# abowman6/CBET_RayTracing_3D

Hardware: AMD Instinct MI355X
Metric: ray-steps/sec, OMEGA 60-beam 256^3 sweep (higher is better)
Workload: dtype f64

## Files before the change

### cbet_raytracing_3d_amd/csrc/cbet_relocate.h

```cpp
#ifndef CBET_RELOCATE_H_
#define CBET_RELOCATE_H_

#include <math.h>

#include "cbet_hd.h"

namespace cbet {

CBET_HD int relocate_loop(int c, double f, int n)
{
    const double half = 0.5001;
    int q = (n - 1 < c + 1) ? n - 1 : c + 1;
    while (q >= ((0 > c - 1) ? 0 : c - 1)) {
        c = (fabs(q - f) < half) ? q : c;
        --q;
    }
    return c;
}

CBET_HD int relocate_closed(int c, double f, int n)
{
    const double half = 0.5001;
    const double fc = (double)c;
    const bool up = (c + 1 <= n - 1) && (fabs((fc + 1.0) - f) < half);
    const bool mid = fabs(fc - f) < half;
    const bool dn1 = (c - 1 >= 0) && (fabs((fc - 1.0) - f) < half);
    const bool dn2 = (c - 2 >= 0) && (fabs((fc - 2.0) - f) < half);
    const int lower = dn1 ? (dn2 ? c - 2 : c - 1) : c;
    const int upper = mid ? c : c + 1;
    return up ? upper : lower;
}

constexpr int kRelocateDeep = 6;
CBET_HD int relocate_deep_interior(int c, double fc, double f, bool &far)
{
    const double half = 0.5001;
    const double g = f - fc;
    far = far || !(fabs(g) < 1.4998);
    return c + ((g >= half) ? 1 : 0) - ((g < (half - 1.0)) ? 1 : 0);
}

}
#endif
```

### cbet_raytracing_3d_amd/csrc/cbet_trace_diag.h

```cpp
#ifndef CBET_TRACE_DIAG_H_
#define CBET_TRACE_DIAG_H_

#include "cbet_trace_common.h"

namespace cbet {

#ifdef CBET_DIAG_CLOCKS
#define CBET_IF_CLOCKS(...) __VA_ARGS__
#else
#define CBET_IF_CLOCKS(...)
#endif
#ifdef CBET_DIAG_FACES
#define CBET_IF_FACES(...) __VA_ARGS__
#else
#define CBET_IF_FACES(...)
#endif
#ifdef CBET_DIAG_CHAIN
#define CBET_IF_CHAIN(...) __VA_ARGS__
#else
#define CBET_IF_CHAIN(...)
#endif

struct WaveDiag {
    typedef unsigned long long u64;
    static constexpr bool kCountsWaveSteps = (0 CBET_IF_CLOCKS(+1) CBET_IF_FACES(+1) CBET_IF_CHAIN(+1)) != 0;
    CBET_IF_CLOCKS(u64 wait = 0, arm = 0, n_arm = 0, ret = 0, n_ret = 0, t_start, t_wait, t_arm, t_ret;)
    CBET_IF_FACES(unsigned near_steps = 0, near_axes = 0, arm_steps = 0;)
    CBET_IF_CHAIN(u64 chain = 0, t_chain = 0;)

    static __device__ __forceinline__ void stamp(u64 &t) { asm volatile("s_memtime %0" : "=&s"(t) : : "memory"); }
    static __device__ __forceinline__ void stamp_wait(u64 &t) { asm volatile("s_memtime %0\n\ts_waitcnt lgkmcnt(0)" : "=&s"(t) : : "memory"); }
    static __device__ __forceinline__ u64 since(u64 t0)
    {
        u64 t1;
        asm volatile("s_memtime %0\n\ts_waitcnt lgkmcnt(0)" : "=&s"(t1) : "s"(t0) : "memory");
        return t1 - t0;
    }

    __device__ __forceinline__ void begin() { CBET_IF_CLOCKS(stamp_wait(t_start);) }
    __device__ __forceinline__ void step_begin(int near)
    {
        (void)near;
        CBET_IF_FACES(near_steps += near != 0 ? 1 : 0; near_axes += __builtin_popcount((unsigned)near);)
    }
    __device__ __forceinline__ void wait_begin() { CBET_IF_CLOCKS(stamp(t_wait);) }
    __device__ __forceinline__ void wait_end()
    {
        CBET_IF_CLOCKS(wait += since(t_wait);)
        CBET_IF_CHAIN(stamp_wait(t_chain);)
    }
    __device__ __forceinline__ void chain_end() { CBET_IF_CHAIN(chain += since(t_chain);) }
    __device__ __forceinline__ void arm_begin()
    {
        CBET_IF_FACES(arm_steps += 1;)
        CBET_IF_CLOCKS(stamp(t_arm);)
    }
    __device__ __forceinline__ void arm_end() { CBET_IF_CLOCKS(arm += since(t_arm); n_arm += 1;) }
    __device__ __forceinline__ void retire_begin() { CBET_IF_CLOCKS(stamp(t_ret);) }
    __device__ __forceinline__ void retire_end() { CBET_IF_CLOCKS(ret += since(t_ret); n_ret += 1;) }
    __device__ __forceinline__ bool report(const TraceArgs &a, int lane, int tot_steps, int tot_rays, unsigned wave_steps)
    {
        auto put = [&](int slot, u64 v) { atomicAdd(&a.counters[slot], v); };
        if (kCountsWaveSteps && lane == 0) {
            CBET_IF_CLOCKS(u64 t_end; stamp_wait(t_end);)
            put(kCntSteps, (u64)tot_steps);
            put(kCntWaveSteps, (u64)wave_steps);
#if defined(CBET_DIAG_CLOCKS)
            put(kCntGlobalAtomics, wait);
            put(kCntEvictions, arm);
            put(kCntWaveStepsWide, n_arm);
            put(kCntSlabsRetired, t_end - t_start);
            put(kCntRays, ret);
            put(kCntWaveStepsMiss, n_ret);
#elif defined(CBET_DIAG_CHAIN)
            put(kCntRays, (u64)tot_rays);
            put(kCntGlobalAtomics, chain);
#elif defined(CBET_DIAG_FACES)
            put(kCntRays, (u64)tot_rays);
            put(kCntWaveStepsWide, (u64)near_steps);
            put(kCntWaveStepsMiss, (u64)near_axes);
            put(kCntSlabsRetired, (u64)arm_steps);
#endif
        }
        (void)tot_rays;
        return kCountsWaveSteps;
    }
};
#undef CBET_IF_CLOCKS
#undef CBET_IF_FACES
#undef CBET_IF_CHAIN

}

#endif
```

### cbet_raytracing_3d_amd/csrc/cbet_trace_window.hip

```cpp
#include <hip/hip_runtime.h>

#include <cstddef>
#include <type_traits>

#if defined(__HIP_DEVICE_COMPILE__) && !defined(__gfx950__)
#error "cbet_trace_window.hip is written for gfx950 (CDNA4) only"
#endif

#include "cbet_trace_common.h"
#include "cbet_trace_diag.h"

namespace cbet {
namespace {

#define CBET_BALLOT(cond) __builtin_amdgcn_ballot_w64(cond)
#define CBET_LANES(mask) __builtin_amdgcn_inverse_ballot_w64(mask)
#define CBET_USUAL(cond) __builtin_expect(!!(cond), 1)
#define CBET_RARE(cond) __builtin_expect(!!(cond), 0)
#define CBET_SELDOM(cond) __builtin_expect_with_probability(!!(cond), 0, 0.9)

template <int WX_, int WY_, int WZ_, bool PAD, bool XORSW = false>
struct Tile {
    static constexpr int WX = WX_, WY = WY_, WZ = WZ_;
    static constexpr int XM = WX - 1, YM = WY - 1, ZM = WZ - 1;
    static constexpr bool ROT = PAD && WZ == 16;
    static constexpr int YS = (PAD && !ROT) ? WZ + 1 : WZ;
    static constexpr int XS = (PAD && !ROT) ? WY * YS + 4 : WY * WZ;
    static constexpr bool XOR = ROT && XORSW;
    static __device__ __forceinline__ int zr(int tx, int ty, int tz)
    {
        return XOR ? (tz ^ ((tx & 3) << 2) ^ (ty << 1)) : (ROT ? ((tz + 7 * tx + 3 * ty) & ZM) : tz);
    }
    static_assert(!XOR || (WX == 8 && WY == 8 && WZ == 16), "the swizzle terms are written for the 8 x 8 x 16 box");
    static __device__ __forceinline__ int xterm(int tx) { return __mul24(tx, XS * 8 + 32) & ~0x80; }
    static __device__ __forceinline__ int yterm(int ty) { return __mul24(ty, YS * 8 + 16); }
    static constexpr int N = WX * XS;
    static constexpr int SX = WX - 2, SY = WY - 2, SZ = WZ - 2;
    static constexpr bool BRICK = WZ == 16 && WY == 8;
    static constexpr int DT = WX * WY * WZ;
    static __device__ __forceinline__ int slot_d(int tx, int ty, int tz) { return (tx * WY + ty) * WZ + tz; }
};

struct Origin {
    int x, y, z;
};

template <int M>
__device__ __forceinline__ int abs_in(int o, int r) { return o + ((r - o) & M); }

template <int C>
struct Corner {
    static constexpr int index = C;
    template <class V> static __device__ __forceinline__ V x(V v0, V v1) { return (C & 1) ? v1 : v0; }
    template <class V> static __device__ __forceinline__ V z(V v0, V v1) { return (C & 2) ? v1 : v0; }
    template <class V> static __device__ __forceinline__ V y(V v0, V v1) { return (C & 4) ? v1 : v0; }
};
template <class F>
__device__ __forceinline__ void each_corner(F f)
{
    f(Corner<0>{}); f(Corner<1>{}); f(Corner<2>{}); f(Corner<3>{}); f(Corner<4>{}); f(Corner<5>{}); f(Corner<6>{}); f(Corner<7>{});
}

struct WaveCounters {
    int n_atomics = 0;
    int n_miss = 0;
    unsigned steps_miss = 0;
    unsigned slabs_bsteps = 0;
    int pend = 0;
    [[no_unique_address]] WaveDiag dg;
};
struct PairedMissCounters : WaveCounters {};

constexpr unsigned long long kEvenLanes = 0x5555555555555555ull;
__device__ __forceinline__ unsigned long long pair_owners(unsigned long long hbm_m, int round)
{
    return hbm_m & (round == 0 ? kEvenLanes : ~kEvenLanes);
}
__device__ __forceinline__ unsigned long long pair_lanes(unsigned long long owners, int round)
{
    return owners | (round == 0 ? owners << 1 : owners >> 1);
}
__device__ __forceinline__ int pair_issued(unsigned long long hbm_m)
{
    return (pair_owners(hbm_m, 0) != 0ull ? 4 : 0) + (pair_owners(hbm_m, 1) != 0ull ? 4 : 0);
}
#define CBET_PAIR_DPP " quad_perm:[1,0,3,2] row_mask:0xf bank_mask:0xf bound_ctrl:1"
__device__ __forceinline__ int pair_pick(unsigned long long owners, int mine, int lent)
{
    int r;
    asm volatile("s_nop 1\n\ts_mov_b64 vcc, %1\n\tv_cndmask_b32_dpp %0, %2, %3, vcc" CBET_PAIR_DPP
                 : "=&v"(r) : "s"(owners), "v"(lent), "v"(mine) : "vcc");
    return r;
}
__device__ __forceinline__ void pair_pick(unsigned long long owners, int mine_n, int lent_n, double mine_v, double lent_v, int &n, double &v)
{
    int lo, hi;
    asm volatile("s_nop 1\n\ts_mov_b64 vcc, %3\n\t"
                 "v_cndmask_b32_dpp %0, %4, %5, vcc" CBET_PAIR_DPP "\n\t"
                 "v_cndmask_b32_dpp %1, %6, %7, vcc" CBET_PAIR_DPP "\n\t"
                 "v_cndmask_b32_dpp %2, %8, %9, vcc" CBET_PAIR_DPP
                 : "=&v"(n), "=&v"(lo), "=&v"(hi)
                 : "s"(owners), "v"(lent_n), "v"(mine_n), "v"(__double2loint(lent_v)), "v"(__double2loint(mine_v)),
                   "v"(__double2hiint(lent_v)), "v"(__double2hiint(mine_v))
                 : "vcc");
    v = __hiloint2double(hi, lo);
}

template <bool W32>
struct Grid {
    double *p;
};
template <bool W32>
__device__ __forceinline__ void grid_add(const TraceArgs &a, Grid<W32> g, int node, double v)
{
    if constexpr (W32) global_add(a, reinterpret_cast<double *>(reinterpret_cast<char *>(g.p) + ((unsigned)node * 8u)), v);
    else global_add(a, &g.p[node], v);
}
template <bool W32>
__device__ __forceinline__ void grid_add_far(const TraceArgs &a, Grid<W32> g, long index, double v) { global_add(a, &g.p[index], v); }

template <class G>
__device__ __forceinline__ void write_back(const TraceArgs &a, double *tile, int slot, G edep, int node, double v, WaveCounters &wc)
{
    wc.pend += (CBET_BALLOT(v != 0.0) != 0ull) ? 1 : 0;
    if (v != 0.0) {
        tile[slot] = 0.0;
        ++wc.n_atomics;
        grid_add(a, edep, node, v);
    }
}
template <class G>
__device__ __forceinline__ void write_back_far(const TraceArgs &a, double *tile, int slot, G edep, long index, double v, WaveCounters &wc)
{
    wc.pend += (CBET_BALLOT(v != 0.0) != 0ull) ? 1 : 0;
    if (v != 0.0) {
        grid_add_far(a, edep, index, v);
        tile[slot] = 0.0;
        ++wc.n_atomics;
    }
}

template <class WC, class F>
__device__ __forceinline__ void miss_add8(unsigned long long hbm_m, WC &wc, F add8)
{
    constexpr bool PAIRED = std::is_same<WC, PairedMissCounters>::value;
    if (CBET_RARE(hbm_m != 0ull)) {
        wc.pend += PAIRED ? pair_issued(hbm_m) : 8;
        if (PAIRED || CBET_LANES(hbm_m)) add8();
    }
}

template <class T, int AX, int COUNT, class G>
__device__ __forceinline__ void retire_planes(const TraceArgs &a, double *tile, const Origin &o, int coord, int step,
                                              int lane, G edep, int sXh, int sYh, WaveCounters &wc)
{
    constexpr int WO = AX == 0 ? T::WY : T::WX, OM = WO - 1;
    constexpr int IT = (WO * T::WZ + kWave - 1) / kWave;
    constexpr int RS = kWave / T::WZ;
    static_assert(IT == 1 || (IT == 2 && 2 * RS == WO), "a plane is one entry per lane, or two in the halves of the other axis");
    static_assert(!T::XOR || IT == 1 || (RS == 4 && T::YS == 16 && T::XS == 128), "the second entry's slot is written for the 8 x 8 x 16 box");
    constexpr int SLOT_X = AX == 0 ? (RS * T::YS) ^ ((2 * RS) & T::ZM) : RS * T::XS;
    const int r0 = lane / T::WZ, r1 = lane & T::ZM, k = abs_in<T::ZM>(o.z, r1);
    const int d0 = (r0 - (AX == 0 ? o.y : o.x)) & OM, dnode = ((d0 & RS) ? -RS : RS) * (AX == 0 ? sYh : sXh);
    const bool in_plane = !(WO * T::WZ < kWave) || lane < WO * T::WZ;
    double v[COUNT * IT];
    int slot[COUNT * IT], node[COUNT * IT];
#pragma unroll
    for (int pl = 0; pl < COUNT; ++pl) {
        const int c = coord + pl * step;
        const int fixed = c & (AX == 0 ? T::XM : T::YM);
#pragma unroll
        for (int e = 0; e < IT; ++e) {
            const int q = pl * IT + e, re = r0 + e * RS;
            if (e == 1 && T::XOR) {
                slot[q] = slot[q - 1] ^ SLOT_X;
                node[q] = node[q - 1] + dnode;
            } else if (AX == 0) {
                slot[q] = fixed * T::XS + re * T::YS + T::zr(fixed, re, r1);
                node[q] = c * sXh + __mul24(abs_in<T::YM>(o.y, re), sYh) + k;
            } else {
                slot[q] = re * T::XS + fixed * T::YS + T::zr(re, fixed, r1);
                node[q] = __mul24(abs_in<T::XM>(o.x, re), sXh) + c * sYh + k;
            }
            const bool ok = in_plane && CBET_AUDIT(a, (unsigned)slot[q] < (unsigned)T::N);
            v[q] = ok ? tile[slot[q]] : 0.0;
        }
    }
#pragma unroll
    for (int q = 0; q < COUNT * IT; ++q) write_back(a, tile, slot[q], edep, node[q], v[q], wc);
}

template <class T, int AX, int NC, class G>
__device__ __forceinline__ void retire_plane(const TraceArgs &a, double *tile, const Origin &o, int coord, int lane,
                                             G edep, int sXh, int sYh, WaveCounters &wc, int coff, long gstride)
{
    constexpr int WO = AX == 0 ? T::WY : T::WX;
    constexpr int IT = (WO * T::WZ + kWave - 1) / kWave;
    const int fixed = coord & (AX == 0 ? T::XM : T::YM);
#pragma unroll
    for (int e = 0; e < IT; ++e) {
        const int idx = e * kWave + lane;
        const bool in_plane = !(WO * T::WZ < kWave) || idx < WO * T::WZ;
        const int r0 = idx / T::WZ, r1 = idx & T::ZM;
        int slot, node, slot_d;
        const int k = abs_in<T::ZM>(o.z, r1);
        if (AX == 0) {
            slot = fixed * T::XS + r0 * T::YS + T::zr(fixed, r0, r1);
            slot_d = T::slot_d(fixed, r0, r1);
            node = coord * sXh + __mul24(abs_in<T::YM>(o.y, r0), sYh) + k;
        } else {
            slot = r0 * T::XS + fixed * T::YS + T::zr(r0, fixed, r1);
            slot_d = T::slot_d(r0, fixed, r1);
            node = __mul24(abs_in<T::XM>(o.x, r0), sXh) + coord * sYh + k;
        }
        const bool ok = in_plane && CBET_AUDIT(a, (unsigned)slot < (unsigned)T::N);
        const double v = ok ? tile[slot] : 0.0;
        if (NC > 1) {
#pragma unroll
            for (int q = 1; q < NC; ++q) {
                const int sq = coff + (q - 1) * T::DT + slot_d;
                write_back_far(a, tile, sq, edep, q * gstride + node, ok ? tile[sq] : 0.0, wc);
            }
        }
        write_back(a, tile, slot, edep, node, v, wc);
    }
}

template <class T, int NC, class G>
__device__ __forceinline__ void retire_zplane(const TraceArgs &a, double *tile, const Origin &o, int coord, int lane,
                                              G edep, int sXh, int sYh, WaveCounters &wc, int coff, long gstride)
{
    static_assert(T::WX * T::WY <= kWave, "one z-plane entry per lane");
    const int r0 = lane / T::WY, r1 = lane & T::YM, fixed = coord & T::ZM;
    const int slot = r0 * T::XS + r1 * T::YS + T::zr(r0, r1, fixed);
    const int node = __mul24(abs_in<T::XM>(o.x, r0), sXh) + __mul24(abs_in<T::YM>(o.y, r1), sYh) + coord;
    const bool ok = (!(T::WX * T::WY < kWave) || lane < T::WX * T::WY) && CBET_AUDIT(a, (unsigned)slot < (unsigned)T::N);
    const double v = ok ? tile[slot] : 0.0;
    if (NC > 1) {
        const int slot_d = T::slot_d(r0, r1, fixed);
#pragma unroll
        for (int q = 1; q < NC; ++q) {
            const int sq = coff + (q - 1) * T::DT + slot_d;
            write_back_far(a, tile, sq, edep, q * gstride + node, ok ? tile[sq] : 0.0, wc);
        }
    }
    write_back(a, tile, slot, edep, node, v, wc);
}

template <class T, class G>
__device__ __forceinline__ void retire_zbrick(const TraceArgs &a, double *tile, const Origin &o, int zb, int lane,
                                              G edep, int sXh, int sYh, WaveCounters &wc)
{
    static_assert(T::WY == 8 && T::WZ == 16, "a brick is 8 rows of 8 planes per tile x index");
    const int ty = lane >> 3, kz = lane & 7;
    const int tz = (zb + kz) & T::ZM;
    const int base_node = __mul24(abs_in<T::YM>(o.y, ty), sYh) + zb + kz;
    constexpr int ROUND = 4;
#pragma unroll
    for (int t0 = 0; t0 < T::WX; t0 += ROUND) {
        double v[ROUND];
        int slot[ROUND];
#pragma unroll
        for (int q = 0; q < ROUND; ++q) {
            slot[q] = (t0 + q) * T::XS + ty * T::YS + T::zr(t0 + q, ty, tz);
            v[q] = CBET_AUDIT(a, (unsigned)slot[q] < (unsigned)T::N) ? tile[slot[q]] : 0.0;
        }
#pragma unroll
        for (int q = 0; q < ROUND; ++q) write_back(a, tile, slot[q], edep, abs_in<T::XM>(o.x, t0 + q) * sXh + base_node, v[q], wc);
    }
}

template <class T, int NC, class G>
__device__ __forceinline__ void flush_box(const TraceArgs &a, double *tile, const Origin &o, int lane, G edep,
                                          int sXh, int sYh, WaveCounters &wc, int coff, long gstride)
{
    for (int t = 0; t < T::WX; ++t)
        retire_plane<T, 0, NC>(a, tile, o, o.x + t, lane, edep, sXh, sYh, wc, coff, gstride);
}

__device__ __forceinline__ int follow_plane_axis(int r, unsigned long long mm, int S)
{
    const unsigned long long edge = __builtin_amdgcn_ballot_w64((unsigned)(r - 1) >= (unsigned)(S - 1)) & mm;
    if (CBET_USUAL(edge == 0ull)) return 0;
    const unsigned long long hi = __builtin_amdgcn_ballot_w64(r >= S) & edge;
    const bool at_hi = hi != 0ull, at_lo = hi != edge;
    if (at_hi == at_lo) return 0;
    if (at_hi) {
        if ((__builtin_amdgcn_ballot_w64(r <= 1) & mm) != 0ull) return (__builtin_amdgcn_ballot_w64(r > S) & mm) != 0ull ? 1 : 0;
        return (S >= 6 && (__builtin_amdgcn_ballot_w64(r <= 2) & mm) == 0ull) ? 2 : 1;
    }
    if ((__builtin_amdgcn_ballot_w64(r >= S - 1) & mm) != 0ull) return (__builtin_amdgcn_ballot_w64(r < 0) & mm) != 0ull ? -1 : 0;
    return (S >= 6 && (__builtin_amdgcn_ballot_w64(r >= S - 2) & mm) == 0ull) ? -2 : -1;
}

__device__ __forceinline__ int follow_brick_axis(int r, unsigned long long mm)
{
    if ((__builtin_amdgcn_ballot_w64((unsigned)r > 14u) & mm) == 0ull) return 0;
    const bool below = (__builtin_amdgcn_ballot_w64(r < 0) & mm) != 0ull, above = (__builtin_amdgcn_ballot_w64(r > 14) & mm) != 0ull;
    const bool needs_lo = (__builtin_amdgcn_ballot_w64(r <= 7) & mm) != 0ull, needs_hi = (__builtin_amdgcn_ballot_w64(r >= 7) & mm) != 0ull;
    return (below && !needs_hi) ? -1 : ((above && !needs_lo) ? 1 : 0);
}

template <class T, int NC, class G>
__device__ __forceinline__ bool follow_box(const TraceArgs &a, double *tile, Origin &o, unsigned long long mm, int lx,
                                           int ly, int lz, int lane, G edep, int sXh, int sYh, WaveCounters &wc,
                                           int coff, long gstride)
{
    auto leave = [&](auto axis, int d, int lo, int hi) {
        constexpr int AX = decltype(axis)::value;
        const int first = d < 0 ? hi : lo, step = d < 0 ? -1 : 1, n = d < 0 ? -d : d;
        if constexpr (NC == 1) {
            if (n == 2) retire_planes<T, AX, 2>(a, tile, o, first, step, lane, edep, sXh, sYh, wc);
            else retire_planes<T, AX, 1>(a, tile, o, first, step, lane, edep, sXh, sYh, wc);
        } else {
            for (int q = 0; q < n; ++q) retire_plane<T, AX, NC>(a, tile, o, first + q * step, lane, edep, sXh, sYh, wc, coff, gstride);
        }
    };
    const int dx = follow_plane_axis(lx - o.x, mm, T::SX);
    const int dy = follow_plane_axis(ly - o.y, mm, T::SY);
    if (dx != 0) { wc.dg.retire_begin(); leave(std::integral_constant<int, 0>{}, dx, o.x, o.x + T::WX - 1); wc.dg.retire_end(); }
    o.x += dx;
    if (dy != 0) { wc.dg.retire_begin(); leave(std::integral_constant<int, 1>{}, dy, o.y, o.y + T::WY - 1); wc.dg.retire_end(); }
    o.y += dy;
    int dz;
    if constexpr (T::BRICK) {
        dz = 8 * follow_brick_axis(lz - o.z, mm);
        if (dz != 0) { wc.dg.retire_begin(); retire_zbrick<T>(a, tile, o, dz < 0 ? o.z + 8 : o.z, lane, edep, sXh, sYh, wc); wc.dg.retire_end(); }
    } else {
        dz = follow_plane_axis(lz - o.z, mm, T::SZ);
        if (dz != 0)
            retire_zplane<T, NC>(a, tile, o, dz < 0 ? o.z + T::WZ - 1 : o.z, lane, edep, sXh, sYh, wc, coff, gstride);
        for (int q = 1; q < (dz < 0 ? -dz : dz); ++q)
            retire_zplane<T, NC>(a, tile, o, dz < 0 ? o.z + T::WZ - 1 - q : o.z + q, lane, edep, sXh, sYh, wc, coff, gstride);
    }
    o.z += dz;
    const bool moved = (dx | dy | dz) != 0;
    wc.slabs_bsteps += moved ? (1u << 16) : 0u;
    return moved;
}

template <class T>
__device__ __forceinline__ bool holds(const Origin &o, int lx, int ly, int lz)
{
    return (unsigned)(lx - o.x) <= (unsigned)T::SX && (unsigned)(ly - o.y) <= (unsigned)T::SY &&
           (unsigned)(lz - o.z) <= (unsigned)T::SZ;
}

template <class T>
__device__ __forceinline__ int box_near_axes(const Origin &o, int nx, int ny, int nz)
{
    const int lo = kRelocateDeep + 1;
    const unsigned tx = (unsigned)((o.x - lo) | (nx - 3 - T::SX - o.x)), ty = (unsigned)((o.y - lo) | (ny - 3 - T::SY - o.y)),
                   tz = (unsigned)((o.z - lo) | (nz - 3 - T::SZ - o.z));
    return (int)((tx >> 31) | ((ty >> 31) << 1) | ((tz >> 31) << 2));
}

typedef double dbl2 __attribute__((ext_vector_type(2)));

template <bool WIDE>
__device__ __forceinline__ void record_issue(const StepRecord *base, unsigned cell, dbl2 &kxy, dbl2 &kzk)
{
    if constexpr (WIDE) {
        const char *p = reinterpret_cast<const char *>(base) + ((unsigned long long)cell << 5);
        asm volatile("global_load_dwordx4 %0, %2, off\n\tglobal_load_dwordx4 %1, %2, off offset:16\n\t; CBET_RECORD_ISSUE %0 %1"
                     : "=&v"(kxy), "=&v"(kzk)
                     : "v"(p)
                     : "memory");
    } else {
        const unsigned off = cell << 5;
        asm volatile("s_nop 4\n\tglobal_load_dwordx4 %0, %2, %3\n\tglobal_load_dwordx4 %1, %2, %3 offset:16\n\t; CBET_RECORD_ISSUE %0 %1"
                     : "=&v"(kxy), "=&v"(kzk)
                     : "v"(off), "s"(base)
                     : "memory");
    }
}

__device__ __forceinline__ void record_wait(dbl2 &kxy, dbl2 &kzk, int pend)
{
    asm volatile("; CBET_RECORD_WAIT %0 %1\n\t"
                 "s_cmp_eq_u32 %2, 0\n\t"
                 "s_cbranch_scc1 .Lrw_0_%=\n\t"
                 "s_cmp_ge_u32 %2, 8\n\t"
                 "s_cbranch_scc1 .Lrw_8_%=\n\t"
                 "s_cmp_ge_u32 %2, 4\n\t"
                 "s_cbranch_scc1 .Lrw_4_%=\n\t"
                 "s_cmp_ge_u32 %2, 2\n\t"
                 "s_cbranch_scc1 .Lrw_2_%=\n\t"
                 "s_waitcnt vmcnt(1)\n\t"
                 "s_branch .Lrw_end_%=\n"
                 ".Lrw_2_%=:\n\t"
                 "s_waitcnt vmcnt(2)\n\t"
                 "s_branch .Lrw_end_%=\n"
                 ".Lrw_4_%=:\n\t"
                 "s_waitcnt vmcnt(4)\n\t"
                 "s_branch .Lrw_end_%=\n"
                 ".Lrw_8_%=:\n\t"
                 "s_waitcnt vmcnt(8)\n\t"
                 "s_branch .Lrw_end_%=\n"
                 ".Lrw_0_%=:\n\t"
                 "s_waitcnt vmcnt(0)\n"
                 ".Lrw_end_%=:"
                 : "+v"(kxy), "+v"(kzk)
                 : "s"(pend)
                 : "memory", "scc");
}

__device__ __forceinline__ void record_wait_all(dbl2 &kxy, dbl2 &kzk)
{
    asm volatile("; CBET_RECORD_WAIT %0 %1\n\ts_waitcnt vmcnt(0)" : "+v"(kxy), "+v"(kzk) : : "memory");
}

__device__ __forceinline__ void exit_planes_load(dbl2 &bx, dbl2 &by, dbl2 &bz)
{
    const void *args = (const void *)__builtin_amdgcn_kernarg_segment_ptr();
    asm volatile("s_load_dwordx4 %0, %3, %4\n\ts_load_dwordx4 %1, %3, %5\n\ts_load_dwordx4 %2, %3, %6\n\ts_waitcnt lgkmcnt(0)"
                 : "=&s"(bx), "=&s"(by), "=&s"(bz)
                 : "s"(args), "i"(offsetof(TraceArgs, exit_planes)), "i"(offsetof(TraceArgs, exit_planes) + 16),
                   "i"(offsetof(TraceArgs, exit_planes) + 32));
}

__device__ __forceinline__ int add3(int a, int b, int c)
{
    int r;
    asm("v_add3_u32 %0, %1, %2, %3" : "=v"(r) : "v"(a), "v"(b), "v"(c));
    return r;
}

__device__ __forceinline__ int xad1(int f, int c)
{
    int r;
    asm("v_xad_u32 %0, %1, 1, %2" : "=v"(r) : "v"(f), "v"(c));
    return r;
}

__device__ __forceinline__ double max_abs3(double a, double b, double c)
{
    double r;
    asm("v_max_f64 %0, |%1|, |%2|" : "=v"(r) : "v"(a), "v"(b));
    asm("v_max_f64 %0, %1, |%2|" : "=v"(r) : "v"(r), "v"(c));
    return r;
}

__device__ __forceinline__ void commit(int &var, int value)
{
    asm volatile("s_mov_b32 %0, %1" : "+s"(var) : "s"(__builtin_amdgcn_readfirstlane(value)));
}
__device__ __forceinline__ void commit(unsigned long long &var, unsigned long long value)
{
    asm volatile("s_mov_b64 %0, %1" : "+s"(var) : "s"(value));
}
__device__ __forceinline__ void commit_v(int &var, int value) { asm volatile("v_mov_b32 %0, %1" : "+v"(var) : "v"(value)); }

__device__ __forceinline__ void cell_step(int &c, unsigned long long up, unsigned long long dn)
{
    asm("s_nop 1\n\tv_addc_co_u32_e64 %0, vcc, 0, %0, %1\n\tv_subbrev_co_u32_e64 %0, vcc, 0, %0, %2" : "+v"(c) : "s"(up), "s"(dn) : "vcc");
}
__device__ __forceinline__ void cell_step3(int &ci, int &cj, int &ck, unsigned long long upx, unsigned long long dnx,
                                           unsigned long long upy, unsigned long long dny, unsigned long long upz,
                                           unsigned long long dnz)
{
    asm("s_nop 1\n\t"
        "v_addc_co_u32_e64 %0, vcc, 0, %0, %3\n\tv_addc_co_u32_e64 %1, vcc, 0, %1, %5\n\tv_addc_co_u32_e64 %2, vcc, 0, %2, %7\n\t"
        "v_subbrev_co_u32_e64 %0, vcc, 0, %0, %4\n\tv_subbrev_co_u32_e64 %1, vcc, 0, %1, %6\n\tv_subbrev_co_u32_e64 %2, vcc, 0, %2, %8"
        : "+v"(ci), "+v"(cj), "+v"(ck)
        : "s"(upx), "s"(dnx), "s"(upy), "s"(dny), "s"(upz), "s"(dnz)
        : "vcc");
}

__device__ __forceinline__ int mad24(int a, int b, int c)
{
    int r;
    asm("s_nop 1\n\tv_mad_i32_i24 %0, %1, %2, %3" : "=v"(r) : "v"(a), "s"(b), "v"(c));
    return r;
}


#ifdef CBET_DEBUG_BOUNDS
constexpr bool kAudited = true;
#else
constexpr bool kAudited = false;
#endif
constexpr double kNearTol = 0.5001;
constexpr double kFarJump = 1.4998;

template <int WZ, bool GENERIC, int CBET, bool STATS>
__global__ void __launch_bounds__(kWave, (CBET == 4) ? 1 : 4) k_trace_window(const TraceArgs a)
{
    using T = Tile<8, 8, WZ, true, CBET == 0>;
    using TB = Tile<4, 8, 8, false>;
    constexpr bool IDX64 = GENERIC;
    constexpr int NC = (CBET == 4) ? 4 : 1;
    constexpr bool ACC = (CBET == 0);
    constexpr bool PIPE = ACC;
    constexpr int NSLOT = T::N + TB::N;
    constexpr int NLDS = NSLOT + (NC - 1) * T::DT;
    __shared__ double s_val[NLDS];
    const int lane = threadIdx.x;

    int beam, patch;
    if (!work_item(a, blockIdx.x, beam, patch)) return;
    const Grid<!IDX64> edep{a.edep + (long)(beam - a.grid_beam0) * a.grid_stride};
    const bool absorb = GENERIC ? (a.absorption == 1) : true;

    Ray s = {};
    int li;
    const bool launched = launch_lane(a, beam, patch, lane, s, li);
    unsigned long long live = __ballot(launched);
    if (live == 0ull) return;
    const int tot_rays = __popcll(live);

    const int nx = a.nx, ny = a.ny, nz = a.nz;
    const int sYh = a.sYh, sXh = a.sXh;
    unsigned cell = launched ? (unsigned)((s.ci * ny + s.cj) * nz + s.ck) : 0u;
    double fcx = (double)s.ci, fcy = (double)s.cj, fcz = (double)s.ck;
    int tot_steps = 0;
    typename std::conditional<CBET == 0, PairedMissCounters, WaveCounters>::type wc;

    double *const tileA = s_val, *const tileB = s_val + T::N;
    Origin oA{0, 0, 0}, oB{0, 0, 0};
    unsigned long long hbm = 0ull;
    int b_active = 0;
    {
        const int src = ((live >> 27) & 1ull) ? 27 : (__ffsll((long long)live) - 1);
        for (int z = lane; z < NLDS; z += kWave) s_val[z] = 0.0;
        oA.x = __builtin_amdgcn_readlane(s.ci, src) + 1 - T::WX / 2;
        oA.y = __builtin_amdgcn_readlane(s.cj, src) + 1 - T::WY / 2;
        oA.z = __builtin_amdgcn_readlane(s.ck, src) + 1 - 4;
        if (T::BRICK) oA.z &= ~7;
        __syncthreads();
    }
    int near = 7;
    wc.dg.begin();

    dbl2 rec_kxy, rec_kzk;
    const StepRecord *rec_base = a.steprec;
    asm volatile("" : "+s"(rec_base));
    double dt = a.dt;
    auto gather_record = [&]() {
        unsigned c = CBET_LANES(live) ? cell : 0u;
        asm("" : "+v"(c));
#ifdef CBET_DEBUG_BOUNDS
        if (!(c < a.audit_nodes)) { audit_fail(a); c = 0u; }
#endif
        record_issue<IDX64>(rec_base, c, rec_kxy, rec_kzk);
        wc.pend = 0;
    };
    auto await_record = [&]() {
        wc.dg.wait_begin();
        if (CBET == 0 && !kAudited) record_wait(rec_kxy, rec_kzk, wc.pend);
        else record_wait_all(rec_kxy, rec_kzk);
        wc.dg.wait_end();
    };
    gather_record();
    await_record();
    const double *const gk = CBET && a.gain ? a.gain + (long)(beam - a.grid_beam0) * a.hsize : nullptr;
    double gained = 0.0;

    const bool flx = (lane & 1) != 0, fly = (lane & 2) != 0, flz = (lane & 8) != 0;
    const int pfx = flx ? 1 : 0, pfy = fly ? 1 : 0, pfz = flz ? 1 : 0;

    double q0 = 0.0, q1 = 0.0, q2 = 0.0, q3 = 0.0;

    int slow = 7;
    double Fx0 = 0, Fx1 = 0, Fy0 = 0, Fy1 = 0, Fz0 = 0, Fz1 = 0;
    int X0 = 0, X1 = 0, Y0 = 0, Y1 = 0, Z0 = 0, Z1 = 0;
    double inc = 0.0;
    int tile_off = 0;
    unsigned long long miss_m = 0ull;
    int own_slot = 0, own_node = 0;
    auto lds_add8 = [&](const double *w) {
        auto add = [&](int byte, double v) {
            if (CBET_AUDIT(a, (unsigned)byte < (unsigned)NSLOT * 8u))
                __hip_atomic_fetch_add(static_cast<double *>(__builtin_assume_aligned(reinterpret_cast<char *>(s_val) + byte, 8)),
                                       v, __ATOMIC_RELAXED, __HIP_MEMORY_SCOPE_WORKGROUP);
        };
        if constexpr (T::XOR) {
            int ax0, ax1, by0, by1, cz0, cz1;
            if (CBET_USUAL(b_active == 0)) {
                ax0 = T::xterm(X0 & T::XM); ax1 = T::xterm(X1 & T::XM);
                by0 = T::yterm(Y0 & T::YM); by1 = T::yterm(Y1 & T::YM);
                cz0 = (Z0 & T::ZM) << 3; cz1 = (Z1 & T::ZM) << 3;
            } else {
                const bool toB = tile_off != 0;
                const int xm = toB ? TB::XM : T::XM, zm = toB ? TB::ZM : T::ZM;
                const int xmul = toB ? TB::XS * 8 : T::XS * 8 + 32, ymul = toB ? TB::YS * 8 : T::YS * 8 + 16;
                const int keep = toB ? ~0 : ~0x80, off8 = tile_off * 8;
                static_assert(TB::YM == T::YM, "one y mask for both boxes");
                ax0 = (__mul24(X0 & xm, xmul) & keep) | off8; ax1 = (__mul24(X1 & xm, xmul) & keep) | off8;
                by0 = __mul24(Y0 & T::YM, ymul); by1 = __mul24(Y1 & T::YM, ymul);
                cz0 = (Z0 & zm) << 3; cz1 = (Z1 & zm) << 3;
            }
            auto at = [](int ax, int by, int cz) { return (int)__builtin_amdgcn_bitop3_b32(ax, by, cz, 0x96); };
            each_corner([=](auto c) { add(at(c.x(ax0, ax1), c.y(by0, by1), c.z(cz0, cz1)), w[c.index]); });
        } else {
            auto add8 = [&](int xm, int ym, int zm, int xs, int ys, int off, int rot) {
                const int xa = X0 & xm, xb = X1 & xm, ya = Y0 & ym, yb = Y1 & ym;
                const int x0 = __mul24(xa, xs * 8) + off * 8, x1 = __mul24(xb, xs * 8) + off * 8;
                const int y0 = __mul24(ya, ys * 8), y1 = __mul24(yb, ys * 8);
                const int ra = 7 * xa * rot, rb = 7 * xb * rot, sa = 3 * ya * rot, sb = 3 * yb * rot;
                auto zb = [&](int z, int r) { return ((z + r) & zm) * 8; };
                if constexpr (T::ROT) {
                    const int xy00 = x0 | y0, xy10 = x1 | y0, xy01 = x0 | y1, xy11 = x1 | y1, zm8 = zm * 8;
                    auto at = [&](int xy, int z, int r) { return (((z + r) * 8) & zm8) | xy; };
                    each_corner([&](auto c) {
                        add(at(c.y(c.x(xy00, xy10), c.x(xy01, xy11)), c.z(Z0, Z1), c.x(ra, rb) + c.y(sa, sb)), w[c.index]);
                    });
                } else {
                    each_corner([&](auto c) {
                        add(add3(c.x(x0, x1), c.y(y0, y1), zb(c.z(Z0, Z1), c.x(ra, rb) + c.y(sa, sb))), w[c.index]);
                    });
                }
            };
            if (b_active == 0) {
                add8(T::XM, T::YM, T::ZM, T::XS, T::YS, 0, T::ROT ? 1 : 0);
            } else {
                const bool toB = tile_off != 0;
                add8(toB ? TB::XM : T::XM, toB ? TB::YM : T::YM, toB ? TB::ZM : T::ZM, toB ? TB::XS : T::XS,
                     toB ? TB::YS : T::YS, tile_off, (T::ROT && !toB) ? 1 : 0);
            }
        }
    };
    auto hbm_add8 = [&](const double *w, unsigned long long hbm_m) {
        const int nX0 = __mul24(X0, sXh), nX1 = __mul24(X1, sXh), nY0 = __mul24(Y0, sYh), nY1 = __mul24(Y1, sYh);
        if constexpr (CBET == 0) {
#pragma unroll
            for (int round = 0; round < 2; ++round) {
                const unsigned long long owners = pair_owners(hbm_m, round);
                if (owners == 0ull) continue;
                const unsigned long long lanes = pair_lanes(owners, round);
                const int z = pair_pick(owners, Z0, Z1);
                each_corner([&](auto c) {
                    if constexpr ((decltype(c)::index & 2) == 0) {
                        const int xy = c.x(nX0, nX1) + c.y(nY0, nY1);
                        int nxy;
                        double v;
                        pair_pick(owners, xy, xy, w[c.index], w[c.index ^ 2], nxy, v);
                        if (CBET_LANES(lanes)) grid_add(a, edep, nxy + z, v);
                    }
                });
            }
            if (CBET_LANES(hbm_m)) wc.n_atomics += 8;
        } else {
            each_corner([&](auto c) { grid_add(a, edep, c.x(nX0, nX1) + c.y(nY0, nY1) + c.z(Z0, Z1), w[c.index]); });
            wc.n_atomics += 8;
        }
    };

    auto deposit_step = [&](unsigned long long lds_m, unsigned long long hbm_m) {
        const double zi0 = Fz0 * inc, zi1 = Fz1 * inc;
        const double zy00 = zi0 * Fy0, zy10 = zi1 * Fy0, zy01 = zi0 * Fy1, zy11 = zi1 * Fy1;
        double wgt[8];
        wgt[0] = zy00 * Fx0;
        wgt[1] = zy00 * Fx1;
        wgt[2] = zy10 * Fx0;
        wgt[3] = zy10 * Fx1;
        wgt[4] = zy01 * Fx0;
        wgt[5] = zy01 * Fx1;
        wgt[6] = zy11 * Fx0;
        wgt[7] = zy11 * Fx1;
        if (CBET_LANES(lds_m)) lds_add8(wgt);
        miss_add8(hbm_m, wc, [&]() {
            hbm_add8(wgt, hbm_m);
            ++wc.n_miss;
        });
        if (CBET == 4) {
            const bool inbox = CBET_LANES(lds_m);
            if (inbox && tile_off == 0) {
                if (CBET_AUDIT(a, (unsigned)(own_slot + 2 * T::DT) < (unsigned)NLDS)) {
                    __hip_atomic_fetch_add(&s_val[own_slot], q1, __ATOMIC_RELAXED, __HIP_MEMORY_SCOPE_WORKGROUP);
                    __hip_atomic_fetch_add(&s_val[own_slot + T::DT], q2, __ATOMIC_RELAXED, __HIP_MEMORY_SCOPE_WORKGROUP);
                    __hip_atomic_fetch_add(&s_val[own_slot + 2 * T::DT], q3, __ATOMIC_RELAXED, __HIP_MEMORY_SCOPE_WORKGROUP);
                }
            } else if (inbox || CBET_LANES(hbm_m)) {
                grid_add_far(a, edep, a.comp_stride + own_node, q1);
                grid_add_far(a, edep, 2 * a.comp_stride + own_node, q2);
                grid_add_far(a, edep, 3 * a.comp_stride + own_node, q3);
                wc.n_atomics += 3;
            }
        }
    };

    double S[8] = {0, 0, 0, 0, 0, 0, 0, 0};
    unsigned long long restart_m = 0ull;
    bool p_odd = true;
    auto accumulate = [&]() {
        const double zi0 = Fz0 * inc, zi1 = Fz1 * inc;
        const double zy00 = zi0 * Fy0, zy10 = zi1 * Fy0, zy01 = zi0 * Fy1, zy11 = zi1 * Fy1;
        const double k = CBET_LANES(restart_m) ? 0.0 : 1.0;
        auto add = [&](double &sum, double w) { asm("v_fma_f64 %0, %0, %1, %2" : "+v"(sum) : "v"(k), "v"(w)); };
        add(S[0], zy00 * Fx0);
        add(S[1], zy00 * Fx1);
        add(S[2], zy10 * Fx0);
        add(S[3], zy10 * Fx1);
        add(S[4], zy01 * Fx0);
        add(S[5], zy01 * Fx1);
        add(S[6], zy11 * Fx0);
        add(S[7], zy11 * Fx1);
    };
    auto flush_sums = [&](unsigned long long lds_m, unsigned long long hbm_m) {
        if (CBET_LANES(lds_m)) lds_add8(S);
        miss_add8(hbm_m, wc, [&]() { hbm_add8(S, hbm_m); });
    };

    auto step_tail = [&](int &tt) {
    asm volatile("" : "+v"(Fx0), "+v"(Fx1), "+v"(Fy0), "+v"(Fy1), "+v"(Fz0), "+v"(Fz1));
    await_record();
    if (absorb) {
        inc = rec_kzk.y * s.uray;
        s.uray -= inc;
    } else {
        inc = s.uray;
    }
    if (CBET >= 2) inc = q0;
    if constexpr (ACC && !PIPE) accumulate();
    unsigned long long died = CBET_BALLOT(s.uray <= s.ustop);
    const int faces = slow | near;
    if (CBET_RARE(faces != 0)) {
        dbl2 bx, by, bz;
        exit_planes_load(bx, by, bz);
        if (faces & 1) died |= CBET_BALLOT(s.px < bx.x) | CBET_BALLOT(s.px > bx.y);
        if (faces & 2) died |= CBET_BALLOT(s.py < by.x) | CBET_BALLOT(s.py > by.y);
        if (faces & 4) died |= CBET_BALLOT(s.pz < bz.x) | CBET_BALLOT(s.pz > bz.y);
    }
    died &= live;
    if (CBET_SELDOM(died != 0ull)) {
        asm volatile("");
        commit(tot_steps, tot_steps + __popcll(died) * (tt + 1));
        if constexpr (PIPE) {
            accumulate();
            asm volatile("v_mov_b64 %0, 0" : "+v"(inc));
            commit(restart_m, 0ull);
        }
        if constexpr (ACC) flush_sums(died & ~miss_m, died & miss_m);
        else deposit_step(died & ~miss_m, died & miss_m);
        commit(live, live & ~died);
        commit(hbm, hbm & live);
        commit(miss_m, miss_m & live);
        if (live == 0ull) commit(tt, a.nt - 1);
    }
    __builtin_amdgcn_wave_barrier();
    };

    for (int tt = 0; tt < a.nt; ++tt) {
        if constexpr (STATS || WaveDiag::kCountsWaveSteps) wc.steps_miss += 1u << 16;
        wc.dg.step_begin(near);
        s.vx -= rec_kxy.x;
        s.vy -= rec_kxy.y;
        s.vz -= rec_kzk.x;
        asm volatile("" : "+s"(dt));
        s.px += s.vx * dt;
        s.py += s.vy * dt;
        s.pz += s.vz * dt;
        const double fx = (s.px - a.xmin) * a.inv_dx;
        const double fy = (s.py - a.ymin) * a.inv_dy;
        const double fz = (s.pz - a.zmin) * a.inv_dz;
        const double g0x = fx - fcx, g0y = fy - fcy, g0z = fz - fcz;
        const unsigned long long upx = CBET_BALLOT(g0x >= kNearTol), dnx = CBET_BALLOT(g0x < kNearTol - 1.0),
                                 upy = CBET_BALLOT(g0y >= kNearTol), dny = CBET_BALLOT(g0y < kNearTol - 1.0),
                                 upz = CBET_BALLOT(g0z >= kNearTol), dnz = CBET_BALLOT(g0z < kNearTol - 1.0);
        slow = ((CBET_BALLOT(!(max_abs3(g0x, g0y, g0z) < kFarJump)) & live) != 0ull) ? 7 : near;
        if (CBET_USUAL(slow == 0)) {
            cell_step3(s.ci, s.cj, s.ck, upx, dnx, upy, dny, upz, dnz);
        } else {
            if (slow & 1) s.ci = relocate_closed(s.ci, fx, nx);
            else cell_step(s.ci, upx, dnx);
            if (slow & 2) s.cj = relocate_closed(s.cj, fy, ny);
            else cell_step(s.cj, upy, dny);
            if (slow & 4) s.ck = relocate_closed(s.ck, fz, nz);
            else cell_step(s.ck, upz, dnz);
        }
        const unsigned new_cell = (unsigned)mad24(mad24(s.ci, ny, s.cj), nz, s.ck);
        unsigned long long moved_m = 0ull;
        if constexpr (ACC) moved_m = CBET_BALLOT(new_cell != cell);
        cell = new_cell;
        gather_record();
        wc.dg.chain_end();
        asm volatile("" : "+v"(s.ci), "+v"(s.cj), "+v"(s.ck), "+v"(inc));
        fcx = (double)s.ci;
        fcy = (double)s.cj;
        fcz = (double)s.ck;
        if constexpr (!ACC) deposit_step(live & ~miss_m, miss_m);
        if constexpr (PIPE) accumulate();
        const double ox = (fx - fcx) - 0.5, oy = (fy - fcy) - 0.5, oz = (fz - fcz) - 0.5;
        const bool ngx = ox < 0, ngy = oy < 0, ngz = oz < 0;
        const bool all_negative = (live & ~(CBET_BALLOT(ngx) & CBET_BALLOT(ngy) & CBET_BALLOT(ngz))) == 0ull;
        if constexpr (ACC) {
            const unsigned long long fl_m = (all_negative && !p_odd) ? (live & moved_m) : live;
            if (CBET_USUAL(fl_m != 0ull)) {
                if (CBET_USUAL(miss_m == 0ull)) flush_sums(fl_m, 0ull);
                else flush_sums(fl_m & ~miss_m, fl_m & miss_m);
            }
            restart_m = fl_m;
            p_odd = !all_negative;
        }
        factor_pair(ox, pfx, Fx0, Fx1);
        factor_pair(oy, pfy, Fy0, Fy1);
        factor_pair(oz, pfz, Fz0, Fz1);
        int rx, ry, rz;
        if (CBET_USUAL(all_negative)) {
            rx = s.ci - oA.x;
            ry = s.cj - oA.y;
            rz = s.ck - oA.z;
            asm("" : "+v"(rx), "+v"(ry), "+v"(rz));
            X0 = xad1(pfx, s.ci); X1 = s.ci + pfx;
            Y0 = xad1(pfy, s.cj); Y1 = s.cj + pfy;
            Z0 = xad1(pfz, s.ck); Z1 = s.ck + pfz;
        } else {
            const int lx = s.ci + 1 - (ngx ? 1 : 0);
            const int ly = s.cj + 1 - (ngy ? 1 : 0);
            const int lz = s.ck + 1 - (ngz ? 1 : 0);
            rx = lx - oA.x;
            ry = ly - oA.y;
            rz = lz - oA.z;
            const bool hx = ngx != flx, hy = ngy != fly, hz = ngz != flz;
            X0 = lx + (hx ? 1 : 0); X1 = lx + (hx ? 0 : 1);
            Y0 = ly + (hy ? 1 : 0); Y1 = ly + (hy ? 0 : 1);
            Z0 = lz + (hz ? 1 : 0); Z1 = lz + (hz ? 0 : 1);
        }
        if (CBET && CBET_LANES(live)) {
            double ds = 0.0;
            if (gk || CBET >= 2) ds = sqrt_speed(__builtin_fma(s.vz, s.vz, __builtin_fma(s.vy, s.vy, s.vx * s.vx))) * a.dt;
            double u_eff = s.uray;
            if (gk) {
                const double x = gain_exponent<IDX64>(a, gk, X0, X1, Y0, Y1, Z0, Z1, Fx0, Fx1, Fy0, Fy1, Fz0, Fz1, sXh, sYh, ds);
                const double phi = gain_phi(x, (CBET_BALLOT(!(fabs(x) < kPhiSmallBelow)) & live) == 0ull);
                const double dg = s.uray * (x * phi);
                u_eff = s.uray * phi;
                gained += dg;
                s.uray = s.uray + dg;
            }
            if (CBET == 2) q0 = u_eff * ds;
            if (CBET == 4) {
                q0 = u_eff * ds;
                q1 = u_eff * (s.vx * a.dt);
                q2 = u_eff * (s.vy * a.dt);
                q3 = u_eff * (s.vz * a.dt);
                const int hi = s.ci + 1, hj = s.cj + 1, hk = s.ck + 1;
                own_slot = T::slot_d(hi & T::XM, hj & T::YM, hk & T::ZM) + NSLOT;
                own_node = __mul24(hi, sXh) + __mul24(hj, sYh) + hk;
            }
        }
        const unsigned long long memA = live & ~hbm;
        unsigned long long out_core = memA & ~(CBET_BALLOT((unsigned)rx <= (unsigned)T::SX) & CBET_BALLOT((unsigned)ry <= (unsigned)T::SY) &
                                               CBET_BALLOT((unsigned)rz <= (unsigned)T::SZ));
        if (CBET_RARE(b_active != 0)) {
            asm volatile("");
            if constexpr (STATS) wc.slabs_bsteps += 1u;
            const int abx = oA.x - oB.x, aby = oA.y - oB.y, abz = oA.z - oB.z;
            out_core |= hbm & ~(CBET_BALLOT((unsigned)(rx + abx) <= (unsigned)TB::SX) &
                                CBET_BALLOT((unsigned)(ry + aby) <= (unsigned)TB::SY) &
                                CBET_BALLOT((unsigned)(rz + abz) <= (unsigned)TB::SZ));
            tile_off = CBET_LANES(hbm) ? T::N : 0;
        }
        out_core |= miss_m;
        if (CBET_RARE(out_core != 0ull)) {
            wc.dg.arm_begin();
            const bool alive = CBET_LANES(live);
            int lx = rx + oA.x, ly = ry + oA.y, lz = rz + oA.z;
            asm volatile("" : "+v"(lx), "+v"(ly), "+v"(lz));
            Origin nA = oA, nB = oB;
            unsigned long long n_hbm = hbm, n_miss = 0ull;
            int n_bact = b_active, n_near, n_toff = tile_off;
            follow_box<T, NC>(a, tileA, nA, memA, lx, ly, lz, lane, edep, sXh, sYh, wc, NSLOT, a.comp_stride);
            const unsigned long long lost_mask =
                memA & ~(CBET_BALLOT((unsigned)(lx - nA.x) <= (unsigned)T::SX) & CBET_BALLOT((unsigned)(ly - nA.y) <= (unsigned)T::SY) &
                         CBET_BALLOT((unsigned)(lz - nA.z) <= (unsigned)T::SZ));
            if (CBET_USUAL(lost_mask == 0ull && n_bact == 0)) {
                n_near = box_near_axes<T>(nA, nx, ny, nz);
            } else {
                bool homeB = CBET_LANES(hbm);
                const bool inA = alive && holds<T>(nA, lx, ly, lz);
                const bool lost = alive && !homeB && !inA;
                if (n_bact != 0) {
                    follow_box<TB, 1>(a, tileB, nB, hbm, lx, ly, lz, lane, edep, sXh, sYh, wc, 0, 0);
                } else if (lost_mask != 0ull) {
                    const int src = __ffsll((long long)lost_mask) - 1;
                    const int sx = __builtin_amdgcn_readlane(lx, src), sy = __builtin_amdgcn_readlane(ly, src),
                              sz = __builtin_amdgcn_readlane(lz, src);
                    nB.x = sx - (TB::WX / 2 - 1);
                    nB.y = sy - (TB::WY / 2 - 1);
                    nB.z = sz - TB::SZ / 2;
                    n_bact = 1;
                }
                const bool inB = alive && holds<TB>(nB, lx, ly, lz);
                homeB = homeB || (lost && inB);
                if (alive && homeB && !inB && inA) homeB = false;
                n_hbm = CBET_BALLOT(alive && homeB);
                if (n_hbm == 0ull) {
                    __builtin_amdgcn_wave_barrier();
                    flush_box<TB, 1>(a, tileB, nB, lane, edep, sXh, sYh, wc, 0, 0);
                    n_bact = 0;
                }
                __builtin_amdgcn_wave_barrier();
                const bool useB = alive && homeB && inB;
                n_toff = useB ? T::N : 0;
                n_miss = live & ~CBET_BALLOT(useB || (alive && !homeB && inA));
                if constexpr (STATS) {
                    if (n_miss != 0ull) wc.steps_miss += 1u;
                    if (ACC && CBET_LANES(n_miss)) ++wc.n_miss;
                }
                n_near = n_miss != 0ull ? 7 : (box_near_axes<T>(nA, nx, ny, nz) | (n_bact == 0 ? 0 : box_near_axes<TB>(nB, nx, ny, nz)));
            }
            commit(oA.x, nA.x); commit(oA.y, nA.y); commit(oA.z, nA.z);
            commit(oB.x, nB.x); commit(oB.y, nB.y); commit(oB.z, nB.z);
            commit(hbm, n_hbm); commit(miss_m, n_miss);
            commit(b_active, n_bact); commit(near, n_near);
            commit_v(tile_off, n_toff);
            wc.pend = __builtin_amdgcn_readfirstlane(wc.pend);
            wc.dg.arm_end();
        } else if (CBET_RARE(near != 0)) {
            commit(near, box_near_axes<T>(oA, nx, ny, nz) | (b_active == 0 ? 0 : box_near_axes<TB>(oB, nx, ny, nz)));
        }
        step_tail(tt);
    }
    tot_steps += __popcll(live) * a.nt;

    if constexpr (PIPE) accumulate();
    if constexpr (ACC) flush_sums(live & ~miss_m, live & miss_m);
    else deposit_step(live & ~miss_m, live & miss_m);
    __syncthreads();
    flush_box<T, NC>(a, tileA, oA, lane, edep, sXh, sYh, wc, NSLOT, a.comp_stride);
    if (b_active != 0) flush_box<TB, 1>(a, tileB, oB, lane, edep, sXh, sYh, wc, 0, 0);

    if (CBET && a.beam_gain) {
        double t = gained;
#pragma unroll
        for (int off = 32; off > 0; off >>= 1) t += __shfl_xor(t, off, kWave);
        if (lane == 0 && t != 0.0) atomicAdd(&a.beam_gain[beam], t);
    }
    if (wc.dg.report(a, lane, tot_steps, tot_rays, wc.steps_miss >> 16)) return;
    if constexpr (STATS) {
        const int tot_at = wave_sum(wc.n_atomics), tot_miss = wave_sum(wc.n_miss);
        if (lane == 0) {
            atomicAdd(&a.counters[kCntGlobalAtomics], (unsigned long long)tot_at);
            atomicAdd(&a.counters[kCntEvictions], (unsigned long long)tot_miss);
            atomicAdd(&a.counters[kCntWaveSteps], (unsigned long long)(wc.steps_miss >> 16));
            atomicAdd(&a.counters[kCntWaveStepsMiss], (unsigned long long)(wc.steps_miss & 0xFFFFu));
            atomicAdd(&a.counters[kCntWaveStepsWide], (unsigned long long)(wc.slabs_bsteps & 0xFFFFu));
            atomicAdd(&a.counters[kCntSlabsRetired], (unsigned long long)(wc.slabs_bsteps >> 16));
        }
    }
    if (lane == 0) {
        atomicAdd(&a.counters[kCntSteps], (unsigned long long)tot_steps);
        atomicAdd(&a.counters[kCntRays], (unsigned long long)tot_rays);
    }
}

}

hipError_t launch_trace_window(const TraceArgs &a, bool force_idx64, hipStream_t stream)
{
    const long waves = a.item_count;
    if (waves <= 0) return hipSuccess;
    const dim3 grid((unsigned)waves), block(kWave);
    const unsigned long long grid_bytes = 8ull * (unsigned long long)a.sXh * (unsigned long long)(a.nx + 2);
    const bool generic = force_idx64 || (a.gain && 8ull * (unsigned long long)a.hsize >= (1ull << 32)) || a.absorption != 1 ||
                         grid_bytes >= (1ull << 32) ||
                         sizeof(StepRecord) * (unsigned long long)a.nx * a.ny * a.nz > (1ull << 32);
    auto go = [&](auto wz, auto cbet) {
        constexpr int WZ = decltype(wz)::value, CB = decltype(cbet)::value;
        if (a.stats) {
            if (generic) hipLaunchKernelGGL((k_trace_window<WZ, true, CB, true>), grid, block, 0, stream, a);
            else hipLaunchKernelGGL((k_trace_window<WZ, false, CB, true>), grid, block, 0, stream, a);
        } else {
            if (generic) hipLaunchKernelGGL((k_trace_window<WZ, true, CB, false>), grid, block, 0, stream, a);
            else hipLaunchKernelGGL((k_trace_window<WZ, false, CB, false>), grid, block, 0, stream, a);
        }
    };
    using std::integral_constant;
    if (a.quantity == 1) go(integral_constant<int, 8>{}, integral_constant<int, 4>{});
    else if (a.quantity == 2) go(integral_constant<int, 16>{}, integral_constant<int, 2>{});
    else if (a.gain || a.beam_gain) go(integral_constant<int, 16>{}, integral_constant<int, 1>{});
    else go(integral_constant<int, 16>{}, integral_constant<int, 0>{});
    return hipGetLastError();
}

}
```

Measured before the change: 178.6 billion.

## Defer dying-ray flush into next pipelined step and refine near-axis mask on misses

When rays die under the pipelined accumulator, the extra accumulate, inc reset and flush_sums on the rare death path are dropped. Dying lanes are instead carried in a mask and folded into the next step's regular flush, so their sums leave through the common path. Separately, on a miss the near-face mask is no longer forced to all three axes. It is computed per axis from the missing lanes' cell positions, which should avoid needless boundary checks. This adds mask bookkeeping and a small correctness risk around miss_m and the final flush of dying lanes. It also adds a diagnostic counter for death events.

```diff
diff --git a/cbet_raytracing_3d_amd/csrc/cbet_relocate.h b/cbet_raytracing_3d_amd/csrc/cbet_relocate.h
--- a/cbet_raytracing_3d_amd/csrc/cbet_relocate.h
+++ b/cbet_raytracing_3d_amd/csrc/cbet_relocate.h
@@ -40,5 +40,14 @@
     return c + ((g >= half) ? 1 : 0) - ((g < (half - 1.0)) ? 1 : 0);
 }
 
+CBET_HD bool cell_near_axis(int c, int n)
+{
+    return n - 3 < kRelocateDeep || (unsigned)(c - kRelocateDeep) > (unsigned)(n - 3 - kRelocateDeep);
+}
+CBET_HD int cell_near_axes(int ci, int cj, int ck, int nx, int ny, int nz)
+{
+    return (cell_near_axis(ci, nx) ? 1 : 0) | (cell_near_axis(cj, ny) ? 2 : 0) | (cell_near_axis(ck, nz) ? 4 : 0);
+}
+
 }
 #endif
diff --git a/cbet_raytracing_3d_amd/csrc/cbet_trace_diag.h b/cbet_raytracing_3d_amd/csrc/cbet_trace_diag.h
--- a/cbet_raytracing_3d_amd/csrc/cbet_trace_diag.h
+++ b/cbet_raytracing_3d_amd/csrc/cbet_trace_diag.h
@@ -25,7 +25,7 @@
     typedef unsigned long long u64;
     static constexpr bool kCountsWaveSteps = (0 CBET_IF_CLOCKS(+1) CBET_IF_FACES(+1) CBET_IF_CHAIN(+1)) != 0;
     CBET_IF_CLOCKS(u64 wait = 0, arm = 0, n_arm = 0, ret = 0, n_ret = 0, t_start, t_wait, t_arm, t_ret;)
-    CBET_IF_FACES(unsigned near_steps = 0, near_axes = 0, arm_steps = 0;)
+    CBET_IF_FACES(unsigned near_steps = 0, near_axes = 0, arm_steps = 0, ended_steps = 0;)
     CBET_IF_CHAIN(u64 chain = 0, t_chain = 0;)
 
     static __device__ __forceinline__ void stamp(u64 &t) { asm volatile("s_memtime %0" : "=&s"(t) : : "memory"); }
@@ -56,6 +56,7 @@
         CBET_IF_CLOCKS(stamp(t_arm);)
     }
     __device__ __forceinline__ void arm_end() { CBET_IF_CLOCKS(arm += since(t_arm); n_arm += 1;) }
+    __device__ __forceinline__ void ended() { CBET_IF_FACES(ended_steps += 1;) }
     __device__ __forceinline__ void retire_begin() { CBET_IF_CLOCKS(stamp(t_ret);) }
     __device__ __forceinline__ void retire_end() { CBET_IF_CLOCKS(ret += since(t_ret); n_ret += 1;) }
     __device__ __forceinline__ bool report(const TraceArgs &a, int lane, int tot_steps, int tot_rays, unsigned wave_steps)
@@ -80,6 +81,7 @@
             put(kCntWaveStepsWide, (u64)near_steps);
             put(kCntWaveStepsMiss, (u64)near_axes);
             put(kCntSlabsRetired, (u64)arm_steps);
+            put(kCntEvictions, (u64)ended_steps);
 #endif
         }
         (void)tot_rays;
diff --git a/cbet_raytracing_3d_amd/csrc/cbet_trace_window.hip b/cbet_raytracing_3d_amd/csrc/cbet_trace_window.hip
--- a/cbet_raytracing_3d_amd/csrc/cbet_trace_window.hip
+++ b/cbet_raytracing_3d_amd/csrc/cbet_trace_window.hip
@@ -682,6 +682,7 @@
 
     double S[8] = {0, 0, 0, 0, 0, 0, 0, 0};
     unsigned long long restart_m = 0ull;
+    unsigned long long dying_m = 0ull;
     bool p_odd = true;
     auto accumulate = [&]() {
         const double zi0 = Fz0 * inc, zi1 = Fz1 * inc;
@@ -726,16 +727,15 @@
     if (CBET_SELDOM(died != 0ull)) {
         asm volatile("");
         commit(tot_steps, tot_steps + __popcll(died) * (tt + 1));
+        wc.dg.ended();
         if constexpr (PIPE) {
-            accumulate();
-            asm volatile("v_mov_b64 %0, 0" : "+v"(inc));
-            commit(restart_m, 0ull);
-        }
-        if constexpr (ACC) flush_sums(died & ~miss_m, died & miss_m);
-        else deposit_step(died & ~miss_m, died & miss_m);
+            commit(dying_m, died);
+        } else {
+            deposit_step(died & ~miss_m, died & miss_m);
+        }
         commit(live, live & ~died);
         commit(hbm, hbm & live);
-        commit(miss_m, miss_m & live);
+        if constexpr (!PIPE) commit(miss_m, miss_m & live);
         if (live == 0ull) commit(tt, a.nt - 1);
     }
     __builtin_amdgcn_wave_barrier();
@@ -785,13 +785,17 @@
         const bool ngx = ox < 0, ngy = oy < 0, ngz = oz < 0;
         const bool all_negative = (live & ~(CBET_BALLOT(ngx) & CBET_BALLOT(ngy) & CBET_BALLOT(ngz))) == 0ull;
         if constexpr (ACC) {
-            const unsigned long long fl_m = (all_negative && !p_odd) ? (live & moved_m) : live;
+            const unsigned long long fl_m = ((all_negative && !p_odd) ? (live & moved_m) : live) | dying_m;
             if (CBET_USUAL(fl_m != 0ull)) {
                 if (CBET_USUAL(miss_m == 0ull)) flush_sums(fl_m, 0ull);
                 else flush_sums(fl_m & ~miss_m, fl_m & miss_m);
             }
             restart_m = fl_m;
             p_odd = !all_negative;
+            if (CBET_RARE(dying_m != 0ull)) {
+                commit(miss_m, miss_m & live);
+                commit(dying_m, 0ull);
+            }
         }
         factor_pair(ox, pfx, Fx0, Fx1);
         factor_pair(oy, pfy, Fy0, Fy1);
@@ -899,7 +903,11 @@
                     if (n_miss != 0ull) wc.steps_miss += 1u;
                     if (ACC && CBET_LANES(n_miss)) ++wc.n_miss;
                 }
-                n_near = n_miss != 0ull ? 7 : (box_near_axes<T>(nA, nx, ny, nz) | (n_bact == 0 ? 0 : box_near_axes<TB>(nB, nx, ny, nz)));
+                n_near = box_near_axes<T>(nA, nx, ny, nz) | (n_bact == 0 ? 0 : box_near_axes<TB>(nB, nx, ny, nz));
+                if (n_miss != 0ull)
+                    n_near |= ((CBET_BALLOT(cell_near_axis(s.ci, nx)) & n_miss) != 0ull ? 1 : 0) |
+                              ((CBET_BALLOT(cell_near_axis(s.cj, ny)) & n_miss) != 0ull ? 2 : 0) |
+                              ((CBET_BALLOT(cell_near_axis(s.ck, nz)) & n_miss) != 0ull ? 4 : 0);
             }
             commit(oA.x, nA.x); commit(oA.y, nA.y); commit(oA.z, nA.z);
             commit(oB.x, nB.x); commit(oB.y, nB.y); commit(oB.z, nB.z);
@@ -916,7 +924,7 @@
     tot_steps += __popcll(live) * a.nt;
 
     if constexpr (PIPE) accumulate();
-    if constexpr (ACC) flush_sums(live & ~miss_m, live & miss_m);
+    if constexpr (ACC) flush_sums((live | dying_m) & ~miss_m, (live | dying_m) & miss_m);
     else deposit_step(live & ~miss_m, live & miss_m);
     __syncthreads();
     flush_box<T, NC>(a, tileA, oA, lane, edep, sXh, sYh, wc, NSLOT, a.comp_stride);
```

New measurement: 178.3 billion, median of 5. About the same (-0.2%).
